# coreperf/rejit

Measured on AMD Instinct MI355X. Metric: GB/s text scanned (regexdna 9 patterns, 50M-line input); matches/s alongside, higher is better.
Workload: dtype u8

## Files before the change

rejit_amd/csrc/kernels.h:

```cpp
#ifndef REJIT_AMD_KERNELS_H_
#define REJIT_AMD_KERNELS_H_

#include <hip/hip_runtime.h>
#include <stdint.h>

#include "dense_streams.h"
#include "device_program.h"
#include "run_scan.h"

namespace rejit_amd {

enum { kCntCands = 0, kCntFinal = 1, kCntOverflow = 2, kCntAdjacent = 3, kCntHits = 4, kCntMaxRegion = 5, kCntOverrun = 6,
  kCntUnordered = 7,
  kCntConflict = 8,
  kCntSharedMax = 9,
  kCntLongWalks = 10,
  kCntSlowStarts = 11,
  kCntSize = 12 };
constexpr uint32_t kOgcMaxBlocks = 256;
constexpr size_t kCounterBlockWords = kCntSize + 2 * kOgcMaxBlocks;
static_assert(kCntLongWalks - kCntOverrun == kLongWalksAfterOverrun, "rj_lane_longest finds the long-walk counter behind the overrun flag");

constexpr uint64_t kNoMatch = ~0ull;

// ... 106 lines not shown
  int n_lists;
  const uint64_t* spans[kMaxFused];
  uint64_t count[kMaxFused];
};
void launch_first_last(const BoundsParams& a, uint64_t* pinned_bounds, hipStream_t st);
void launch_bounds_rows(const BoundsParams& a, int64_t offset, int first_round, int64_t* d_rows, hipStream_t st);
void launch_carry_decide(const int64_t* d_all, int world, int rank, int n_patterns, int64_t* out, hipStream_t st);
void launch_globalize_spans(const uint64_t* local, uint64_t count, int64_t offset, uint64_t* out, hipStream_t st);
void launch_scan_windows_fused(const FusedParams& a, int grid, hipEvent_t t0, hipEvent_t t1, hipStream_t st);

struct PlaneParams {
  const uint8_t* text;
  uint64_t n;
  uint64_t sb, se;
  uint64_t span_pairs;
  uint32_t offset;
  uint32_t code_shift;
  uint32_t n_bases;
  uint32_t lo[2][8], hi[2][8];
  uint64_t* hits;
  uint32_t region_cap;
  uint32_t* hit_counts;
  uint32_t n_zero;
  unsigned long long* zero_counters[kMaxFused];
};
void launch_plane_scan(const PlaneParams& a, int grid, hipEvent_t t0, hipEvent_t t1, hipStream_t st);

enum { kPcConflict = 1,
       kPcVoid = 2 };
constexpr uint32_t kPcBounds = 0;
constexpr uint32_t kPcTotals = kPcBounds + 64;
constexpr uint32_t kPcFinishGroups = 8;
constexpr uint32_t kPcTicket = kPcTotals + 32;
constexpr uint32_t kPcGroupRows = kPcTicket + 16;
constexpr uint32_t kPcAccWords = kPcGroupRows + kPcFinishGroups * 96;
constexpr uint32_t kPcHostCount = 0, kPcHostFlags = 32, kPcHostBounds = 40, kPcHostWords = 40 + 64;
constexpr unsigned long long kPcNone = ~0ull;
constexpr uint32_t kPcLenShift = 56;
struct PlaneCountParams {
  const uint8_t* text;
  uint64_t n;
  uint64_t sb, se;
  uint64_t first_block, end_block;
  uint64_t span_blocks;
  uint32_t span_extra;
  uint32_t code_shift, n_bases, n_patterns;
  uint32_t batch_at;
  uint32_t mask_bits;
  uint32_t base_lo[2], base_hi[2];
  const uint32_t* table;
  uint32_t table_words;
  unsigned long long* acc;
  uint32_t* wg_rows;
  unsigned long long* wg_bounds;
  unsigned long long* host_out;
};
void launch_plane_count(const PlaneCountParams& a, int grid, hipEvent_t t0, hipEvent_t t1, hipStream_t st);
struct PlaneListParams {
  PlaneCountParams c;
  uint64_t* hits;
  uint32_t region_cap;
  uint32_t offset;
  uint32_t* hit_counts;
  uint32_t n_zero;
  unsigned long long* zero_counters[kMaxFused];
};
void launch_plane_list(const PlaneListParams& a, int grid, hipEvent_t t0, hipEvent_t t1, hipStream_t st);
void launch_plane_count_finish(const PlaneCountParams& a, int grid, hipStream_t st);
void launch_bounds_rows_counts(const BoundsParams& a, const unsigned long long* acc, int64_t offset, int first_round, int64_t* d_rows, hipStream_t st);

struct StreamParams {
  const uint8_t* text;
  uint64_t n;
  uint64_t sb, se;
  uint64_t first_tile, n_tiles;
  unsigned long long* granules;
  unsigned long long* ticket;
  uint64_t* out;
  uint64_t out_cap;
  unsigned long long* counters;
  unsigned long long* host_counters;
  uint32_t max_walk;
  StreamPlan plan;
};
uint64_t stream_tiles(uint64_t sb, uint64_t se, uint64_t n, uint64_t* first_tile);
size_t stream_scratch_bytes(uint64_t n_tiles);
void launch_dense_streams(StreamParams a, unsigned long long* scratch, hipEvent_t t0, hipEvent_t t1, hipStream_t st);

constexpr uint64_t kRunTile = 8192;
struct RunSummary {
// ... 209 lines not shown
```

rejit_amd/csrc/multi_pattern.hip:

```cpp

#include <cstring>
#include <dlfcn.h>

#include <hip/hip_runtime.h>

#include <algorithm>
#include <chrono>
#include <cstdio>
#include <cstdlib>
#include <memory>
#include <mutex>
#include <string>
#include <thread>
#include <vector>

#include "engine_internal.h"
#include "exact_count.h"

using namespace rejit_amd;

#define fail ::rejit_amd::rj_fail

namespace {

// ... 250 lines not shown
  bool classify_tables_ready = false;
  DeviceBuffer dummy_counts;
  DeviceBuffer tails;
  MultiTail* host_tails = nullptr;
  uint64_t* host_bounds = nullptr;
  hipStream_t second = nullptr;
  hipEvent_t fork = nullptr, join = nullptr;
  std::vector<MultiTail> uploaded;
  bool fused = false;
  bool batchable = false;
  int mode = 0;
  float scan_ms = 0.f;
  struct Pending {
    bool active = false;
    int kind = 0;
    const uint8_t* text = nullptr;
    uint64_t n = 0, sb = 0, se = 0;
    hipStream_t st = nullptr;
    bool fuse = false;
    std::vector<uint64_t> caps;
    uint32_t shared_cap = 0;
    hipEvent_t done = nullptr;
  } pending;
  rj_multi* scan_after = nullptr;
  hipStream_t tail_stream = nullptr;
  bool tails_own_stream = false;
  DeviceBuffer exchange_rows;
  int64_t* host_decision = nullptr;
  bool counts_only = false;
  ExactCountPlan exact;
  DeviceBuffer exact_table, count_acc, wg_rows, wg_bounds;
  unsigned long long* count_out = nullptr;
  bool counts_ready = false;
  PlanePlan gplane;
  bool general_counts = false;
  DeviceBuffer count_blob;
  uint32_t count_desc_words = 0, count_blob_words = 0, count_lmax = 0, count_max_short = 0;
  int count_max_words = 1;
  bool count_blob_ready = false;
  bool last_counts = false;
  uint32_t counts_fallbacks = 0;

};

namespace {

SharedHits shared_hits_of(rj_multi* m, const uint8_t* d_text, uint64_t n, uint64_t sb, uint64_t se, uint32_t shared_cap, uint32_t n_regions, int P) {
  SharedHits sh{};
  sh.hits = m->shared_hits.as<uint64_t>();
  sh.counts = m->shared_counts.as<uint32_t>();
  sh.cap = shared_cap;
  sh.n_regions = n_regions;
  sh.n_patterns = static_cast<uint32_t>(P);
  sh.win_offset = m->plane.offset;
  sh.text = d_text;
  sh.n = n;
  sh.sb = sb;
  sh.se = se;
  static const bool forward = getenv("RJ_CLASSIFY_FORWARD") != nullptr;
  sh.reverse = forward ? 0u : 1u;
  return sh;
}

int classify_blob(rj_multi* m, hipStream_t st) {
  const int P = static_cast<int>(m->scans.size());
  if (!m->host_desc) RJ_HIP(hipHostMalloc(reinterpret_cast<void**>(&m->host_desc), sizeof(ClassifyDesc) * kMaxFused));
// ... 566 lines not shown
  RJ_HIP(hipStreamSynchronize(st));
  m->count_blob_ready = true;
  return RJ_OK;
}

int run_spans(rj_multi* m, const uint8_t* d_text, uint64_t n, uint64_t sb, uint64_t se, hipStream_t st) {
  if (m->fused && m->mode == 0 && n >= 16) {
    int rc = run_batched(m, d_text, n, sb, se, st, true);
    if (rc != kRegionsFull) return rc != RJ_OK ? rc : 1;
  } else if (m->batchable && n >= 16) {
    int rc = run_batched(m, d_text, n, sb, se, st, false);
    if (rc != kRegionsFull) return rc != RJ_OK ? rc : 2;
  }
  for (rj_scan* s : m->scans) {
    int rc = run_pipeline(s, d_text, n, sb, se, 0, 0, 0, st);
    if (rc != RJ_OK) return rc;
  }
  return 0;
}

int run_counts(rj_multi* m, const uint8_t* d_text, uint64_t n, uint64_t sb, uint64_t se, hipStream_t st, int phase) {
  const int P = static_cast<int>(m->scans.size());
  rj_scan* const s0 = m->scans[0];
  if (phase != 2) {
    const bool general = !(m->exact.ok && m->plane.ok && !m->plane.general && m->plane.offset == 0);
    const PlanePlan& plan = general ? m->gplane : m->plane;
    const uint32_t cmp = general ? plan.n_cmp : 8u;
    const uint64_t last_w = n >= cmp ? n - cmp + 1 : 0;
    const uint64_t wlo = sb + (general ? plan.min_offset : 0u), whi = std::min<uint64_t>(se + (general ? plan.max_offset : 0u), last_w);
    const uint64_t first_block = wlo / 2048;
    const uint64_t end_block = whi > wlo ? (whi + 2047) / 2048 : first_block;
    const uint64_t blocks = end_block - first_block;
    static const int count_chunks = getenv("RJ_COUNT_CHUNKS") ? atoi(getenv("RJ_COUNT_CHUNKS")) : 128;
    const ScanGeometry geo = scan_geometry(std::max<uint64_t>(blocks * 2, 1), static_cast<uint64_t>(count_chunks > 0 ? count_chunks : 128));
    if (!m->counts_ready) {
      if (!m->count_out) RJ_HIP(hipHostMalloc(reinterpret_cast<void**>(&m->count_out), sizeof(unsigned long long) * kPcHostWords));
      if (m->exact.ok) {
        RJ_HIP(m->exact_table.reserve(sizeof(uint32_t) * kExactTabWords));
        RJ_HIP(hipMemcpyAsync(m->exact_table.p, m->exact.table, sizeof(uint32_t) * kExactTabWords, hipMemcpyHostToDevice, st));
      }
      RJ_HIP(m->count_acc.reserve(sizeof(unsigned long long) * kPcAccWords));
      RJ_HIP(hipMemsetAsync(m->count_acc.p, 0, sizeof(unsigned long long) * kPcAccWords, st));
      m->counts_ready = true;
    }
    PlaneCountParams pc{};
    pc.text = d_text;
    pc.n = n;
    pc.sb = sb;
    pc.se = se;
    pc.first_block = first_block;
    pc.end_block = end_block;
    pc.span_blocks = blocks / geo.n_regions;
    pc.span_extra = static_cast<uint32_t>(blocks % geo.n_regions);
    pc.code_shift = plan.code_shift;
    pc.n_bases = plan.n_bases;
    pc.n_patterns = static_cast<uint32_t>(P);
    static const int batch_at = getenv("RJ_COUNT_BATCH") ? atoi(getenv("RJ_COUNT_BATCH")) : 64;
    pc.batch_at = static_cast<uint32_t>(std::min(std::max(batch_at, 1), 64));
    PlaneCountGParams pg{};
    if (general) {
      int rc = count_blob(m, st);
      if (rc != RJ_OK) return rc;
      pc.table = m->count_blob.as<uint32_t>();
      pc.table_words = m->count_blob_words;
      pg.n_cmp = plan.n_cmp;
      pg.tolerance = plan.tolerance;
      pg.lmax = m->count_lmax;
      pg.desc_words = m->count_desc_words;
      for (uint32_t b = 0; b < kPlaneMaxBases; b++)
        for (uint32_t i = 0; i < 8; i++)
          pg.idx[b][i] = i < plan.n_cmp ? (static_cast<uint32_t>(plan.base[b < plan.n_bases ? b : 0][i]) >> plan.code_shift) & 3u : 4u;
    } else {
      for (uint32_t b = 0; b < 2; b++) {
        const uint32_t bb = b < plan.n_bases ? b : 0;
        for (int i = 0; i < 8; i++) {
          const uint32_t code = (static_cast<uint32_t>(plan.base[bb][i]) >> plan.code_shift) & 3u;
          if (!(code & 1u)) pc.mask_bits |= 1u << (16 * b + 2 * i);
          if (!(code & 2u)) pc.mask_bits |= 1u << (16 * b + 2 * i + 1);
        }
        pc.base_lo[b] = m->exact.base_lo[bb];
        pc.base_hi[b] = m->exact.base_hi[bb];
      }
      pc.table = m->exact_table.as<uint32_t>();
    }
    pc.acc = m->count_acc.as<unsigned long long>();
    pc.host_out = m->count_out;
    RJ_HIP(m->wg_rows.reserve(sizeof(uint32_t) * kExactMaxPatterns * static_cast<size_t>(geo.grid)));
    RJ_HIP(m->wg_bounds.reserve(sizeof(unsigned long long) * 2 * kExactMaxPatterns * static_cast<size_t>(geo.grid)));
    pc.wg_rows = m->wg_rows.as<uint32_t>();
    pc.wg_bounds = m->wg_bounds.as<unsigned long long>();
    if (m->scan_after != nullptr && m->scan_after != m && m->scan_after->scans[0]->ev[2] != nullptr)
      RJ_HIP(hipStreamWaitEvent(st, m->scan_after->scans[0]->ev[2], 0));
    if (general) {
      pg.c = pc;
      launch_plane_count_general(pg, m->count_max_words, m->count_max_short, geo.grid, s0->t0(), s0->ev[2], st);
    } else {
      launch_plane_count(pc, geo.grid, s0->t0(), s0->ev[2], st);
    }
    hipStream_t fs = st;
    if (phase == 1) {
      if (!m->tail_stream) RJ_HIP(hipStreamCreateWithFlags(&m->tail_stream, hipStreamNonBlocking));
      fs = m->tail_stream;
      RJ_HIP(hipStreamWaitEvent(fs, s0->ev[2], 0));
    }
    launch_plane_count_finish(pc, geo.grid, fs);
    if (phase == 1) {
      if (!m->pending.done) RJ_HIP(hipEventCreateWithFlags(&m->pending.done, hipEventDisableTiming));
      RJ_HIP(hipEventRecord(m->pending.done, fs));
      return RJ_OK;
    }
  }
  if (phase == 2) RJ_HIP(hipEventSynchronize(m->pending.done));
  else RJ_HIP(hipStreamSynchronize(st));
  RJ_HIP(hipGetLastError());
  if (m->count_out[kPcHostFlags] != 0) {
    m->counts_fallbacks++;
    m->last_counts = false;
    int kind = run_spans(m, d_text, n, sb, se, st);
    return kind < 0 ? kind : RJ_OK;
  }
  m->scan_ms = 0.f;
  if (s0->timing) (void)hipEventElapsedTime(&m->scan_ms, s0->ev[1], s0->ev[2]);
  for (int p = 0; p < P; p++) {
    rj_scan* s = m->scans[static_cast<size_t>(p)];
    s->stats = rj_stats{};
    s->result = nullptr;
    s->result_count = m->count_out[kPcHostCount + p];
    s->stats.n_matches = s->result_count;
    s->stats.scan_ms = m->scan_ms;
    s->stats.count_path = 1;
// ... 452 lines not shown
int64_t rj_scan_gather_spans(rj_scan* s, const void* d_text, uint64_t n, uint64_t own_begin, uint64_t own_end, int64_t offset, void* rccl_comm, int rank,
                             int world, int root, void* hip_stream) {
  if (!rccl_comm) return fail(RJ_BAD_ARGUMENT, "rj_scan_gather_spans: no communicator");
  if (!rccl().all_gather) return fail(RJ_DEVICE_ERROR, "rj_scan_gather_spans: librccl.so not found (set RJ_RCCL_LIBRARY)");
  RcclGatherCtx c{rccl_comm, rank, world};
  return rj_scan_gather_spans_via(s, d_text, n, own_begin, own_end, offset, rccl_allgather_ctx, rccl_gatherv, &c, rank, world, root, hip_stream);
}

const uint64_t* rj_scan_gathered_spans(const rj_scan* s, uint64_t* count) {
  if (count) *count = s ? s->gathered_count : 0;
  return s ? s->gathered : nullptr;
}

int rj_multi_set_tail_stream(rj_multi* m, int on) {
  ErrnoGuard errno_guard;
  if (!m) return fail(RJ_BAD_ARGUMENT, "null argument");
  if (m->pending.active) return fail(RJ_BAD_ARGUMENT, "rj_multi_set_tail_stream: a run is in flight");
  if (on && !m->tail_stream) RJ_HIP(hipStreamCreateWithFlags(&m->tail_stream, hipStreamNonBlocking));
  m->tails_own_stream = on != 0;
  return RJ_OK;
}

int rj_multi_set_timing(rj_multi* m, int on) {
  if (!m) return fail(RJ_BAD_ARGUMENT, "null argument");
  for (rj_scan* s : m->scans) s->timing = on != 0;
  return RJ_OK;
}

int rj_multi_set_counts_only(rj_multi* m, int on) {
  ErrnoGuard errno_guard;
  if (!m) return fail(RJ_BAD_ARGUMENT, "null argument");
  if (m->pending.active) return fail(RJ_BAD_ARGUMENT, "rj_multi_set_counts_only: a run is in flight");
  m->counts_only = on != 0;
  return (m->counts_only && counts_shape(m)) ? 1 : 0;
}

}

int64_t rejit_amd::scan_count(rj_scan* s, const uint8_t* d_text, uint64_t n, hipStream_t st) {
  s->rec_valid = false;
  if (s->counter_state == 0) {
    s->counter_state = -1;
    const rj_program* progs[1] = {s->prog};
    rj_multi* m = nullptr;
    if (n >= 16 && (fusable(s->prog) || plane_general_ok(s->prog)) && rj_multi_create(progs, 1, &m) == RJ_OK) {
      if (rj_multi_set_counts_only(m, 1) == 1) {
        (void)rj_multi_set_timing(m, s->timing ? 1 : 0);
        s->counter = m;
        s->counter_state = 1;
      } else {
        rj_multi_destroy(m);
      }
    } else if (n < 16) {
      s->counter_state = 0;
    }
  }
  if (s->counter_state == 1 && n >= 16 && (reinterpret_cast<uintptr_t>(d_text) & 15u) == 0) {
    uint64_t count = 0;
    int how = rj_multi_run(s->counter, d_text, n, &count, st);
    if (how < 0) return how;
    rj_scan* inner = s->counter->scans[0];
    s->stats = inner->stats;
    s->result_count = inner->result_count;
    s->result = nullptr;
    if (how != 3) s->stats.count_path = 0;
    return static_cast<int64_t>(count);
// ... 25 lines not shown
```

rejit_amd/csrc/plane_count.hip:

```cpp
#include <hip/hip_runtime.h>
#include <hip/hip_ext.h>

#include <cstdlib>

#include "exact_count.h"
#include "kernels.h"
#include "plane_codes.h"
#include "short_walk.h"
#include "stream_load.h"
#include "wave_ops.h"

namespace rejit_amd {

namespace {

constexpr uint64_t kBlock = 2048;
constexpr uint32_t kPieceB = 1024;
constexpr uint32_t kStashWords = (2048 + 16) / 4;
#ifndef RJ_PC_RING
#define RJ_PC_RING 256
#endif
constexpr uint32_t kRing = RJ_PC_RING;

__device__ __forceinline__ uint32_t codes16(const uint4& v, const PlaneCodes& k) {
// ... 119 lines not shown
        const uint32_t e = E[i][b];
        if (i == 0) {
          Z[b] = e;
        } else if (i == 1) {
          O[b] = Z[b] | e;
          Z[b] &= e;
        } else {
          O[b] = Z[b] | (O[b] & e);
          if (i < 7) Z[b] &= e;
        }
      }
  }
  return NB > 1 ? (O[0] | O[NB - 1]) : O[0];
}


struct Lens {
  uint64_t w[2];
};
static_assert(kMaxFused <= 24, "two words of twelve lengths");
__device__ __forceinline__ uint32_t len_of(const Lens& l, uint32_t p) {
  return static_cast<uint32_t>((p < 12 ? l.w[0] >> (5 * p) : l.w[1] >> (5 * (p - 12))) & 31u);
}

}

template <int NB>
struct ExactShape {
  using Args = PlaneCountParams;
  static constexpr uint32_t kFixedLen = 8;
  static constexpr bool kBlobInLds = false;
  static constexpr bool kList = false;
  static constexpr bool kCapture = true;
  __device__ static __forceinline__ const PlaneCountParams& common(const Args& g) { return g; }
  __device__ static __forceinline__ uint32_t lmax(const Args&) { return 8u; }
  __device__ static __forceinline__ uint32_t offset_of(const Args&, const uint32_t*, uint32_t) { return 0u; }
  __device__ static __forceinline__ uint32_t test(uint32_t ta, uint32_t tb, uint32_t ha, uint32_t hb, const Args& g) { return plane_test<NB>(ta, tb, ha, hb, g); }
  __device__ static __forceinline__ void classify(const Args& a, const uint32_t* table, uint64_t pos, bool have, uint32_t& mask, Lens&) {
    const bool ok = have && pos >= a.sb && pos < a.se && pos + 8 <= a.n;
    uint32_t lo = 0, hi = 0;
    if (ok) {
      __builtin_memcpy(&lo, a.text + pos, 4);
      __builtin_memcpy(&hi, a.text + pos + 4, 4);
    }
    mask = exact_classify<NB>(table, a.base_lo, a.base_hi, lo, hi);
    mask = ok ? mask : 0u;
  }
  __device__ static __forceinline__ void classify_bytes(const Args& a, const uint32_t* table, uint64_t pos, bool have, uint32_t lo, uint32_t hi, uint32_t& mask) {
    const bool ok = have && pos >= a.sb && pos < a.se && pos + 8 <= a.n;
    mask = exact_classify<NB>(table, a.base_lo, a.base_hi, lo, hi);
    mask = ok ? mask : 0u;
  }
};

template <int NB>
struct ListShape {
  using Args = PlaneListParams;
  static constexpr uint32_t kFixedLen = 8;
  static constexpr bool kBlobInLds = false;
  static constexpr bool kList = true;
  static constexpr bool kCapture = false;
  __device__ static __forceinline__ void classify_bytes(const Args&, const uint32_t*, uint64_t, bool, uint32_t, uint32_t, uint32_t& mask) { mask = 0; }
  __device__ static __forceinline__ const PlaneCountParams& common(const Args& g) { return g.c; }
  __device__ static __forceinline__ uint32_t lmax(const Args&) { return 8u; }
  __device__ static __forceinline__ uint32_t offset_of(const Args&, const uint32_t*, uint32_t) { return 0u; }
  __device__ static __forceinline__ uint32_t test(uint32_t ta, uint32_t tb, uint32_t ha, uint32_t hb, const Args& g) { return plane_test<NB>(ta, tb, ha, hb, g.c); }
  __device__ static __forceinline__ void classify(const Args&, const uint32_t*, uint64_t, bool, uint32_t& mask, Lens&) { mask = 0; }
};

namespace {

template <bool TOL>
__device__ __forceinline__ uint32_t general_test(uint32_t ta, uint32_t tb, uint32_t ha, uint32_t hb, const PlaneCountGParams& g) {
  constexpr uint32_t kEven = 0x55555555u;
  const uint32_t L = (ta & kEven) | ((tb << 1) & ~kEven);
  const uint32_t H = ((ta >> 1) & kEven) | (tb & ~kEven);
  const uint32_t Ln = (ha & kEven) | ((hb << 1) & ~kEven);
  const uint32_t Hn = ((ha >> 1) & kEven) | (hb & ~kEven);
  register uint32_t q0 asm("v48") = ~(L | H);
  register uint32_t q1 asm("v49") = L & ~H;
  register uint32_t q2 asm("v50") = ~L & H;
  register uint32_t q3 asm("v51") = L & H;
  register uint32_t q4 asm("v52") = ~0u;
  register uint32_t n0 asm("v56") = ~(Ln | Hn);
  register uint32_t n1 asm("v57") = Ln & ~Hn;
  register uint32_t n2 asm("v58") = ~Ln & Hn;
  register uint32_t n3 asm("v59") = Ln & Hn;
  register uint32_t n4 asm("v60") = ~0u;
  uint32_t c = 0;
#pragma clang loop unroll(disable)
  for (uint32_t b = 0; b < g.c.n_bases; b++) {
    const uint32_t* ix = g.idx[b];
    uint32_t e0, e1, e2, e3, e4, e5, e6, e7;
    asm volatile(
// ... 19 lines not shown
          "v"(q3), "v"(q4), "v"(n0), "v"(n1), "v"(n2), "v"(n3), "v"(n4));
    if (TOL) {
      uint32_t Z = e0, O = e0 | e1;
      Z &= e1;
      O = Z | (O & e2);
      Z &= e2;
      O = Z | (O & e3);
      Z &= e3;
      O = Z | (O & e4);
      Z &= e4;
      O = Z | (O & e5);
      Z &= e5;
      O = Z | (O & e6);
      Z &= e6;
      O = Z | (O & e7);
      c |= O;
    } else {
      const uint32_t z0 = e0 & e1 & e2, z1 = e3 & e4 & e5;
      c |= z0 & z1 & e6 & e7;
    }
  }
  return c;
}

}

template <int W, int MAXK, bool TOL>
struct GeneralShape {
  using Args = PlaneCountGParams;
  static constexpr uint32_t kFixedLen = 0;
  static constexpr bool kBlobInLds = true;
  static constexpr bool kList = false;
  static constexpr bool kCapture = false;
  __device__ static __forceinline__ void classify_bytes(const Args&, const uint32_t*, uint64_t, bool, uint32_t, uint32_t, uint32_t& mask) { mask = 0; }
  __device__ static __forceinline__ const PlaneCountParams& common(const Args& g) { return g.c; }
  __device__ static __forceinline__ uint32_t lmax(const Args& g) { return g.lmax; }
  __device__ static __forceinline__ uint32_t offset_of(const Args&, const uint32_t* blob, uint32_t p) {
    return reinterpret_cast<const ClassifyDesc*>(blob)[p].win_offset;
  }
  __device__ static __forceinline__ uint32_t test(uint32_t ta, uint32_t tb, uint32_t ha, uint32_t hb, const Args& g) { return general_test<TOL>(ta, tb, ha, hb, g); }
  __device__ static __forceinline__ void classify(const Args& g, const uint32_t* blob, uint64_t w, bool have, uint32_t& mask, Lens& lens) {
    const PlaneCountParams& a = g.c;
    const ClassifyDesc* desc = reinterpret_cast<const ClassifyDesc*>(blob);
    const uint32_t* tab = blob + g.desc_words;
    uint32_t lo = 0, hi = 0;
    if (have) {
      if (w + 8 <= a.n) {
        __builtin_memcpy(&lo, a.text + w, 4);
        __builtin_memcpy(&hi, a.text + w + 4, 4);
      } else {
        for (uint32_t q = 0; q < 8 && w + q < a.n; q++) {
          const uint32_t c = a.text[w + q];
          if (q < 4) lo |= c << (8 * q);
          else hi |= c << (8 * (q - 4));
        }
      }
    }
    uint32_t todo = 0;
    for (uint32_t p = 0; p < a.n_patterns; p++) {
      const ClassifyDesc& d = desc[p];
      const uint64_t s = w - d.win_offset;
      const bool ok = have && w >= d.win_offset && s >= a.sb && s < a.se && w + d.win_len <= a.n;
      bool win = false;
      for (uint32_t q = 0; q < d.n_windows; q++) win = win || ((((lo ^ d.v0[q]) & d.m0[q]) | ((hi ^ d.v1[q]) & d.m1[q])) == 0);
      todo |= (ok && win) ? 1u << p : 0u;
    }
    mask = 0;
    lens.w[0] = lens.w[1] = 0;
    while (__ballot(todo != 0) != 0) {
      const bool act = todo != 0;
      const uint32_t p = act ? static_cast<uint32_t>(__builtin_ctz(todo)) : 0u;
      todo &= todo - 1;
      const ClassifyDesc& d = desc[p];
      const uint32_t* t0 = tab + d.tab;
      const uint64_t s = w - d.win_offset;
      uint64_t t_lo = 0, t_hi = 0;
      if (act) rj_load16(a.text, a.n, s, &t_lo, &t_hi);
      const uint32_t avail = act ? (a.n - s < 16 ? static_cast<uint32_t>(a.n - s) : 16u) : 0u;
      uint32_t len = 0;
      bool found;
      if (W == 1 || d.n_words <= 1) found = short_longest_lds<1, MAXK>(t0, d, t_lo, t_hi, avail, &len);
      else found = short_longest_lds<W, MAXK>(t0, d, t_lo, t_hi, avail, &len);
      if (found && act && len != 0) {
        mask |= 1u << p;
        if (p < 12) lens.w[0] |= static_cast<uint64_t>(len) << (5 * p);
        else lens.w[1] |= static_cast<uint64_t>(len) << (5 * (p - 12));
      }
    }
  }
};

template <bool TOL>
struct GeneralListShape {
  using Args = PlaneListGParams;
  static constexpr uint32_t kFixedLen = 0;
  static constexpr bool kBlobInLds = false;
  static constexpr bool kList = true;
  static constexpr bool kCapture = false;
  __device__ static __forceinline__ void classify_bytes(const Args&, const uint32_t*, uint64_t, bool, uint32_t, uint32_t, uint32_t& mask) { mask = 0; }
  __device__ static __forceinline__ const PlaneCountParams& common(const Args& g) { return g.g.c; }
  __device__ static __forceinline__ uint32_t lmax(const Args& g) { return g.g.lmax; }
  __device__ static __forceinline__ uint32_t offset_of(const Args&, const uint32_t*, uint32_t) { return 0u; }
  __device__ static __forceinline__ uint32_t test(uint32_t ta, uint32_t tb, uint32_t ha, uint32_t hb, const Args& g) { return general_test<TOL>(ta, tb, ha, hb, g.g); }
  __device__ static __forceinline__ void classify(const Args&, const uint32_t*, uint64_t, bool, uint32_t& mask, Lens&) { mask = 0; }
};

namespace {

struct WaveState {
  uint32_t* ring;
  uint32_t* stash;
  uint32_t head, tail;
  uint32_t acc;
  uint32_t flags;
  uint32_t prev_rel, prev_valid;
  uint32_t* ends;
  uint64_t* list;
  uint32_t list_cap;
  uint64_t list_base;
};
constexpr uint32_t kNoEnd = 0xFFFFFFFFu;

template <bool LIST, bool CAPTURE>
__device__ __forceinline__ void push_block(WaveState& w, uint32_t hm, uint32_t rel_lane, uint32_t block_rel = 0, uint32_t slot = 0) {
  const uint64_t any = __ballot(hm != 0);
  if (any == 0) return;
  auto put = [&](uint32_t idx, uint32_t rel) {
    if (LIST) {
      if (idx < w.list_cap) w.list[idx] = w.list_base + rel;
    } else {
      w.ring[idx & (kRing - 1)] = rel;
// ... 107 lines not shown
  uint32_t any[2] = {0, 0};
#pragma unroll
  for (int round = 0; round < 2; round++) {
    const uint64_t pos = round == 0 ? span_base + static_cast<uint64_t>(lane) - reach : span_base + rel;
    const bool mine = round == 0 ? (static_cast<uint32_t>(lane) < reach && span_base + static_cast<uint64_t>(lane) >= reach) : near;
    uint32_t mask;
    Lens lens;
    S::classify(g, tab, pos, mine, mask, lens);
    for (uint32_t p = 0; p < a.n_patterns; p++)
      if (__ballot(((mask >> p) & 1u) != 0) != 0) any[round] |= 1u << p;
  }
  if ((any[0] & any[1]) != 0) w.flags |= kPcConflict;
}

template <class S>
__device__ __forceinline__ void blocks_done(WaveState& w, const uint32_t* tab, const typename S::Args& g, uint64_t span_base, bool& first_batch) {
  const PlaneCountParams& a = S::common(g);
  if (w.tail - w.head > kRing) {
    w.flags |= kPcVoid;
    w.head = w.tail;
    return;
  }
  while (w.tail - w.head >= a.batch_at) {
    const uint32_t held = w.tail - w.head;
    const uint32_t m = held < 64u ? held : 64u;
    if (first_batch) check_span_start<S>(w, m, tab, g, span_base);
    first_batch = false;
    classify_batch<S>(w, m, tab, g, span_base);
  }
}

}

template <class S>
__global__ __launch_bounds__(256) void plane_count(typename S::Args g) {
  __shared__ __attribute__((aligned(16))) uint32_t table[kExactTabWords];
  extern __shared__ __attribute__((aligned(16))) uint32_t blob[];
  __shared__ uint32_t rings[4][kRing * (S::kCapture ? 3 : 1)];
  __shared__ __attribute__((aligned(16))) uint32_t stashes[4][S::kCapture ? 2 * kStashWords : 4];
  __shared__ uint32_t ends[4][4 * kExactMaxPatterns];
  __shared__ unsigned long long wave_bounds[4][kExactMaxPatterns][2];
  __shared__ uint32_t wave_counts[4][kExactMaxPatterns];
  __shared__ uint32_t wave_flags[4];
  const PlaneCountParams& a = S::common(g);
  const uint32_t* tab = S::kBlobInLds ? blob : table;
  const int lane = lane_id();
  const uint32_t wid = threadIdx.x >> 6;
  const uint32_t wave = __builtin_amdgcn_readfirstlane(static_cast<uint32_t>((static_cast<uint64_t>(blockIdx.x) * blockDim.x + threadIdx.x) >> 6));
  PlaneCodes k;
  k.shift = a.code_shift;
  k.cmask = 0x03030303u << a.code_shift;
  const uint32_t c0 = static_cast<uint32_t>(a.first_block) + wave * static_cast<uint32_t>(a.span_blocks) + (wave < a.span_extra ? wave : a.span_extra);
  const uint32_t c1 = c0 + static_cast<uint32_t>(a.span_blocks) + (wave < a.span_extra ? 1u : 0u);
  const uint32_t full = static_cast<uint32_t>(a.n / kBlock);
  uint32_t fast_end = full >= 1 ? full - 1 : 0;
  if (fast_end > c1) fast_end = c1;
  if (fast_end < c0) fast_end = c0;
  const uint64_t span_base = static_cast<uint64_t>(c0) * kBlock;
  WaveState w;
  w.ring = rings[wid];
  w.stash = stashes[wid];
  w.ends = ends[wid];
  w.head = w.tail = 0;
  w.acc = 0;
  w.flags = 0;
  w.prev_rel = w.prev_valid = 0;
  w.ends[lane] = kNoEnd;
  w.ends[lane + 64] = kNoEnd;
  w.list = nullptr;
  w.list_cap = 0;
  w.list_base = 0;
  if constexpr (S::kList) {
    if (wave == 0 && lane < kCntSize)
      for (uint32_t p = 0; p < g.n_zero; p++) g.zero_counters[p][lane] = 0;
    w.list = g.hits + static_cast<uint64_t>(wave) * g.region_cap;
    w.list_cap = g.region_cap;
    w.list_base = span_base - g.offset;
  }
  bool first_batch = true;

  const uint32_t last_own = fast_end > c0 ? fast_end - 1 : c0;
  auto blk = [&](uint32_t c) { return a.text + static_cast<uint64_t>(c < last_own ? c : last_own) * kBlock; };
  const uint32_t lane_rel = static_cast<uint32_t>(lane) * 16u;
  Raw ra, rb;
  uint2 behind{0, 0};
  uint32_t c = c0;
  auto stash_put = [&](uint32_t ci, const Raw& r) __attribute__((always_inline)) {
    if constexpr (S::kCapture) {
      uint32_t* sl = w.stash + (ci & 1u) * kStashWords;
      *reinterpret_cast<uint4*>(sl + lane * 4) = r.a;
      *reinterpret_cast<uint4*>(sl + kPieceB / 4 + lane * 4) = r.b;
    }
  };
  auto spill_put = [&](uint32_t ci, uint32_t x, uint32_t y) __attribute__((always_inline)) {
    if constexpr (S::kCapture) {
      if (lane == 0) *reinterpret_cast<uint2*>(w.stash + (ci & 1u) * kStashWords + kBlock / 4) = make_uint2(x, y);
    }
  };
  if (c < fast_end) {
    load_block(blk(c), lane_rel, ra);
    load_block(blk(c + 1), lane_rel, rb);
    behind = *reinterpret_cast<const uint2*>(a.text + static_cast<uint64_t>(fast_end) * kBlock);
  }
  if (S::kList) {
  } else if (S::kBlobInLds) {
    const uint4* src = reinterpret_cast<const uint4*>(a.table);
    uint4* dst = reinterpret_cast<uint4*>(blob);
    for (uint32_t i = threadIdx.x; i < a.table_words / 4; i += blockDim.x) dst[i] = src[i];
  } else {
    for (uint32_t i = threadIdx.x; i < kExactTabWords; i += blockDim.x) table[i] = a.table[i];
  }
  __syncthreads();
  if (c < fast_end) {
    uint32_t xa = codes16(ra.a, k), xb = codes16(ra.b, k);
    stash_put(c, ra);
    if (S::kCapture) __builtin_amdgcn_sched_barrier(0);
    load_block(blk(c + 2), lane_rel, ra);
    const uint32_t behind_codes = (codes4(behind.x, k) >> k.shift) | (codes4(behind.y, k) << (8 - k.shift));
    while (c + 1 < fast_end) {
      const uint32_t ya = codes16(rb.a, k), yb = codes16(rb.b, k);
      asm volatile("" ::"v"(ya), "v"(yb));
      stash_put(c + 1, rb);
      spill_put(c, rb.a.x, rb.a.y);
      if (S::kCapture) __builtin_amdgcn_sched_barrier(0);
      if (c + 3 <= last_own) load_block(blk(c + 3), lane_rel, rb);
      {
        const uint32_t ha = wave_from_lane_above(xa, static_cast<uint32_t>(__builtin_amdgcn_readfirstlane(static_cast<int>(xb))));
        const uint32_t hb = wave_from_lane_above(xb, static_cast<uint32_t>(__builtin_amdgcn_readfirstlane(static_cast<int>(ya))));
        const uint32_t hm = S::test(xa, xb, ha, hb, g);
        push_block<S::kList, S::kCapture>(w, hm, (c - c0) * static_cast<uint32_t>(kBlock) + lane_rel, (c - c0) * static_cast<uint32_t>(kBlock), c & 1u);
      }
      __builtin_amdgcn_sched_barrier(0);
      xa = codes16(ra.a, k);
      xb = codes16(ra.b, k);
      asm volatile("" ::"v"(xa), "v"(xb));
      if (c + 2 < fast_end) {
        stash_put(c + 2, ra);
        spill_put(c + 1, ra.a.x, ra.a.y);
      } else {
        spill_put(c + 1, behind.x, behind.y);
      }
      if (S::kCapture) __builtin_amdgcn_sched_barrier(0);
      if (c + 4 <= last_own) load_block(blk(c + 4), lane_rel, ra);
      {
        const uint32_t next0 = c + 2 == fast_end ? behind_codes : static_cast<uint32_t>(__builtin_amdgcn_readfirstlane(static_cast<int>(xa)));
// ... 30 lines not shown
    const uint32_t g0 = guarded_dword(a.text, a.n, at + 16), g1 = guarded_dword(a.text, a.n, at + 20);
    const uint32_t h0 = guarded_dword(a.text, a.n, bt + 16), h1 = guarded_dword(a.text, a.n, bt + 20);
    const uint32_t ha = (codes4(g0, k) >> k.shift) | (codes4(g1, k) << (8 - k.shift));
    const uint32_t hb = (codes4(h0, k) >> k.shift) | (codes4(h1, k) << (8 - k.shift));
    const uint32_t hm = S::test(codes16(va, k), codes16(vb, k), ha, hb, g);
    if (!S::kList && w.tail - w.head > kRing - 64u) blocks_done<S>(w, tab, g, span_base, first_batch);
    if constexpr (S::kCapture) {
      Raw gr;
      gr.a = va;
      gr.b = vb;
      stash_put(c, gr);
      const uint64_t nb = (static_cast<uint64_t>(c) + 1) * kBlock;
      spill_put(c, guarded_dword(a.text, a.n, nb), guarded_dword(a.text, a.n, nb + 4));
    }
    push_block<S::kList, S::kCapture>(w, hm, (c - c0) * static_cast<uint32_t>(kBlock) + lane_rel, (c - c0) * static_cast<uint32_t>(kBlock), c & 1u);
  }
  if constexpr (S::kList) {
    if (lane == 0) g.hit_counts[wave] = w.tail;
    return;
  }
  if (w.tail - w.head > kRing) {
    w.flags |= kPcVoid;
    w.head = w.tail;
  }
  while (w.tail != w.head) {
    const uint32_t held = w.tail - w.head;
    const uint32_t m = held < 64u ? held : 64u;
    if (first_batch) check_span_start<S>(w, m, tab, g, span_base);
    first_batch = false;
    classify_batch<S>(w, m, tab, g, span_base);
  }
  if (lane < kExactMaxPatterns) {
    const bool real = lane < static_cast<int>(a.n_patterns);
    wave_counts[wid][lane] = real ? w.acc : 0u;
    const uint32_t ef = w.ends[4 * lane], efl = w.ends[4 * lane + 1], el = w.ends[4 * lane + 2], ell = w.ends[4 * lane + 3];
    const uint64_t off = real ? S::offset_of(g, tab, static_cast<uint32_t>(lane)) : 0u;
    wave_bounds[wid][lane][0] = ef != kNoEnd ? ((span_base + ef - off) | (static_cast<unsigned long long>(efl) << kPcLenShift)) : kPcNone;
    wave_bounds[wid][lane][1] = ef != kNoEnd ? ((span_base + el - off) | (static_cast<unsigned long long>(ell) << kPcLenShift)) : kPcNone;
  }
  if (lane == 0) wave_flags[wid] = w.flags;
  __syncthreads();
  if (wid != 0 || lane >= kExactMaxPatterns) return;
  uint32_t v = wave_counts[0][lane] + wave_counts[1][lane] + wave_counts[2][lane] + wave_counts[3][lane];
  if (lane == kExactMaxPatterns - 1) v = wave_flags[0] | wave_flags[1] | wave_flags[2] | wave_flags[3];
  a.wg_rows[static_cast<uint64_t>(blockIdx.x) * kExactMaxPatterns + lane] = v;
  if (lane < static_cast<int>(a.n_patterns) && v != 0) {
    unsigned long long first = kPcNone, last = kPcNone;
#pragma unroll
    for (int q = 3; q >= 0; q--)
      if (wave_bounds[q][lane][0] != kPcNone) first = wave_bounds[q][lane][0];
#pragma unroll
    for (int q = 0; q < 4; q++)
      if (wave_bounds[q][lane][1] != kPcNone) last = wave_bounds[q][lane][1];
    *reinterpret_cast<ulonglong2*>(a.wg_bounds + (static_cast<uint64_t>(blockIdx.x) * kExactMaxPatterns + lane) * 2) = ulonglong2{first, last};
  }
}

constexpr uint32_t kFinishBatch = 8;
__global__ __launch_bounds__(256, 8) void plane_count_finish(PlaneCountParams a, uint32_t n_wg) {
  __shared__ unsigned long long part[32][kExactMaxPatterns];
  __shared__ uint32_t part_first[32][kExactMaxPatterns], part_last[32][kExactMaxPatterns];
  __shared__ uint32_t is_last;
  const uint32_t p4 = threadIdx.x & 7u, q = threadIdx.x >> 3;
  const uint32_t per = (n_wg + gridDim.x - 1) / gridDim.x;
  const uint32_t r_lo = blockIdx.x * per, r_hi = r_lo + per < n_wg ? r_lo + per : n_wg;
  uint32_t sum[4] = {0, 0, 0, 0};
  uint32_t first_row[4] = {0, 0, 0, 0}, last_row[4] = {0, 0, 0, 0};
  const uint4* rows = reinterpret_cast<const uint4*>(a.wg_rows);
  for (uint32_t r = r_lo + q; r < r_hi; r += 32 * kFinishBatch) {
    uint4 v[kFinishBatch];
#pragma unroll
    for (uint32_t i = 0; i < kFinishBatch; i++) {
      const uint32_t rr = r + 32 * i;
      v[i] = rows[static_cast<uint64_t>(rr < r_hi ? rr : r) * 8 + p4];
      if (rr >= r_hi) v[i] = uint4{0, 0, 0, 0};
    }
#pragma unroll
    for (uint32_t i = 0; i < kFinishBatch; i++) {
      const uint32_t rr1 = r + 32 * i + 1;
      const uint32_t c[4] = {v[i].x, v[i].y, v[i].z, v[i].w};
      sum[0] += v[i].x;
      sum[1] += v[i].y;
      sum[2] += v[i].z;
      sum[3] = p4 == 7 ? (sum[3] | v[i].w) : (sum[3] + v[i].w);
#pragma unroll
      for (int k = 0; k < 4; k++) {
        first_row[k] = (c[k] != 0 && first_row[k] == 0) ? rr1 : first_row[k];
        last_row[k] = c[k] != 0 ? rr1 : last_row[k];
      }
    }
  }
#pragma unroll
  for (int i = 0; i < 4; i++) {
    part[q][4 * p4 + i] = sum[i];
    part_first[q][4 * p4 + i] = first_row[i];
    part_last[q][4 * p4 + i] = last_row[i];
  }
  __syncthreads();
  const uint32_t lane = threadIdx.x & 63u, wave_id = threadIdx.x >> 6;
  if (wave_id == 0) {
    if (lane < kExactMaxPatterns) {
      unsigned long long t = 0;
      uint32_t f = 0, l = 0;
#pragma unroll 4
      for (uint32_t i = 0; i < 32; i++) {
        t = lane == kExactMaxPatterns - 1 ? (t | part[i][lane]) : (t + part[i][lane]);
        const uint32_t pf = part_first[i][lane], pl = part_last[i][lane];
        f = pf != 0 && (f == 0 || pf < f) ? pf : f;
        l = pl > l ? pl : l;
      }
      unsigned long long* g = a.acc + kPcGroupRows + blockIdx.x * 96;
      __hip_atomic_store(&g[lane], t, __ATOMIC_RELAXED, __HIP_MEMORY_SCOPE_AGENT);
      __hip_atomic_store(&g[32 + lane], static_cast<unsigned long long>(f), __ATOMIC_RELAXED, __HIP_MEMORY_SCOPE_AGENT);
      __hip_atomic_store(&g[64 + lane], static_cast<unsigned long long>(l), __ATOMIC_RELAXED, __HIP_MEMORY_SCOPE_AGENT);
    }
    if (lane == 0) {
      const unsigned long long t = __hip_atomic_fetch_add(&a.acc[kPcTicket], 1ull, __ATOMIC_ACQ_REL, __HIP_MEMORY_SCOPE_AGENT);
      is_last = t + 1 == gridDim.x ? 1u : 0u;
      if (t + 1 == gridDim.x) __hip_atomic_store(&a.acc[kPcTicket], 0ull, __ATOMIC_RELAXED, __HIP_MEMORY_SCOPE_AGENT);
    }
  }
  __syncthreads();
  if (!is_last || threadIdx.x >= kExactMaxPatterns) return;
  const uint32_t p = threadIdx.x;
  unsigned long long total = 0;
  uint32_t f = 0, l = 0;
#pragma unroll 2
  for (uint32_t g = 0; g < gridDim.x; g++) {
    const unsigned long long* row = a.acc + kPcGroupRows + g * 96;
    const unsigned long long v = __hip_atomic_load(&row[p], __ATOMIC_RELAXED, __HIP_MEMORY_SCOPE_AGENT);
    const uint32_t pf = static_cast<uint32_t>(__hip_atomic_load(&row[32 + p], __ATOMIC_RELAXED, __HIP_MEMORY_SCOPE_AGENT));
    const uint32_t pl = static_cast<uint32_t>(__hip_atomic_load(&row[64 + p], __ATOMIC_RELAXED, __HIP_MEMORY_SCOPE_AGENT));
    total = p == kExactMaxPatterns - 1 ? (total | v) : (total + v);
    f = pf != 0 && (f == 0 || pf < f) ? pf : f;
    l = pl > l ? pl : l;
  }
  if (p == kExactMaxPatterns - 1) a.host_out[kPcHostFlags] = total;
  if (p >= a.n_patterns) return;
  unsigned long long first = kPcNone, last = kPcNone;
  if (total != 0 && f != 0) {
    first = a.wg_bounds[(static_cast<uint64_t>(f - 1) * kExactMaxPatterns + p) * 2];
    last = a.wg_bounds[(static_cast<uint64_t>(l - 1) * kExactMaxPatterns + p) * 2 + 1];
  }
  a.host_out[kPcHostCount + p] = total;
  a.host_out[kPcHostBounds + 2 * p] = first;
  a.host_out[kPcHostBounds + 2 * p + 1] = last;
  a.acc[kPcBounds + 2 * p] = first;
  a.acc[kPcBounds + 2 * p + 1] = last;
  a.acc[kPcTotals + p] = total;
}

__global__ void bounds_rows_counts_kernel(BoundsParams a, const unsigned long long* acc, int64_t offset, int first_round, int64_t* rows) {
// ... 4 lines not shown
  if (a.spans[p]) {
    const uint64_t* r = a.spans[p];
    if (n) {
      fb = static_cast<int64_t>(r[0]) + offset;
      fe = static_cast<int64_t>(r[1]) + offset;
      lb = static_cast<int64_t>(r[2 * (n - 1)]) + offset;
      le = static_cast<int64_t>(r[2 * (n - 1) + 1]) + offset;
    }
  } else {
    n = acc[kPcTotals + p];
    if (n) {
      const unsigned long long f = acc[kPcBounds + 2 * p], l = acc[kPcBounds + 2 * p + 1];
      const unsigned long long at = (1ull << kPcLenShift) - 1;
      fb = static_cast<int64_t>(f & at) + offset;
      fe = fb + static_cast<int64_t>(f >> kPcLenShift);
      lb = static_cast<int64_t>(l & at) + offset;
      le = lb + static_cast<int64_t>(l >> kPcLenShift);
    }
  }
  rows[8 * p + 0] = static_cast<int64_t>(n);
  if (first_round) {
    rows[8 * p + 1] = fb;
    rows[8 * p + 2] = fe;
    rows[8 * p + 5] = rows[8 * p + 6] = rows[8 * p + 7] = 0;
  }
  rows[8 * p + 3] = lb;
  rows[8 * p + 4] = le;
}

void launch_bounds_rows_counts(const BoundsParams& a, const unsigned long long* acc, int64_t offset, int first_round, int64_t* d_rows, hipStream_t st) {
  hipLaunchKernelGGL(bounds_rows_counts_kernel, dim3(1), dim3(64), 0, st, a, acc, offset, first_round, d_rows);
}

void launch_plane_count(const PlaneCountParams& a, int grid, hipEvent_t t0, hipEvent_t t1, hipStream_t st) {
  static const size_t pad = getenv("RJ_COUNT_LDS_PAD") ? static_cast<size_t>(atoi(getenv("RJ_COUNT_LDS_PAD"))) : 0;
  if (a.n_bases <= 1) hipExtLaunchKernelGGL((plane_count<ExactShape<1>>), dim3(grid), dim3(256), pad, st, t0, t1, 0, a);
  else hipExtLaunchKernelGGL((plane_count<ExactShape<2>>), dim3(grid), dim3(256), pad, st, t0, t1, 0, a);
}

void launch_plane_list(const PlaneListParams& a, int grid, hipEvent_t t0, hipEvent_t t1, hipStream_t st) {
  if (a.c.n_bases <= 1) hipExtLaunchKernelGGL((plane_count<ListShape<1>>), dim3(grid), dim3(256), 0, st, t0, t1, 0, a);
  else hipExtLaunchKernelGGL((plane_count<ListShape<2>>), dim3(grid), dim3(256), 0, st, t0, t1, 0, a);
}

void launch_plane_list_general(const PlaneListGParams& a, int grid, hipEvent_t t0, hipEvent_t t1, hipStream_t st) {
  if (a.g.tolerance) hipExtLaunchKernelGGL((plane_count<GeneralListShape<true>>), dim3(grid), dim3(256), 0, st, t0, t1, 0, a);
  else hipExtLaunchKernelGGL((plane_count<GeneralListShape<false>>), dim3(grid), dim3(256), 0, st, t0, t1, 0, a);
}

void launch_plane_count_general(const PlaneCountGParams& g, int max_words, uint32_t max_short, int grid, hipEvent_t t0, hipEvent_t t1, hipStream_t st) {
  const size_t lds = static_cast<size_t>(g.c.table_words) * sizeof(uint32_t);
  const dim3 gr(grid), b(256);
  if (g.tolerance) {
    if (max_words <= 1 && max_short <= 8) hipExtLaunchKernelGGL((plane_count<GeneralShape<1, 8, true>>), gr, b, lds, st, t0, t1, 0, g);
    else if (max_words <= 1) hipExtLaunchKernelGGL((plane_count<GeneralShape<1, 16, true>>), gr, b, lds, st, t0, t1, 0, g);
    else hipExtLaunchKernelGGL((plane_count<GeneralShape<2, 16, true>>), gr, b, lds, st, t0, t1, 0, g);
  } else {
    if (max_words <= 1 && max_short <= 8) hipExtLaunchKernelGGL((plane_count<GeneralShape<1, 8, false>>), gr, b, lds, st, t0, t1, 0, g);
    else if (max_words <= 1) hipExtLaunchKernelGGL((plane_count<GeneralShape<1, 16, false>>), gr, b, lds, st, t0, t1, 0, g);
    else hipExtLaunchKernelGGL((plane_count<GeneralShape<2, 16, false>>), gr, b, lds, st, t0, t1, 0, g);
  }
}

void launch_plane_count_finish(const PlaneCountParams& a, int grid, hipStream_t st) {
  hipLaunchKernelGGL(plane_count_finish, dim3(kPcFinishGroups), dim3(256), 0, st, a, static_cast<uint32_t>(grid));
}

}
```

Before: 50230.

## Make exact count kernel persistent with atomic work-unit claiming

The exact plane_count kernel becomes a persistent kernel. Only as many workgroups as fit resident on the device are launched, and each one claims further work units through an atomic counter, double-buffering its per-wave shared reductions across turns. The lookup table is staged into LDS once per workgroup rather than once per unit. The aim is to cut launch and tail cost and to balance load across CUs, at the price of an atomic per unit and a loop with extra state. The claim counter is reset by the finish kernel. Optional env knobs set the unit size, cap the group count, or turn claiming off.

Measured after the change: 41700. -17.0%, worse.

```diff
diff --git a/rejit_amd/csrc/kernels.h b/rejit_amd/csrc/kernels.h
--- a/rejit_amd/csrc/kernels.h
+++ b/rejit_amd/csrc/kernels.h
@@ -162,6 +162,7 @@
 constexpr uint32_t kPcTotals = kPcBounds + 64;
 constexpr uint32_t kPcFinishGroups = 8;
 constexpr uint32_t kPcTicket = kPcTotals + 32;
+constexpr uint32_t kPcClaim = kPcTicket + 8;
 constexpr uint32_t kPcGroupRows = kPcTicket + 16;
 constexpr uint32_t kPcAccWords = kPcGroupRows + kPcFinishGroups * 96;
 constexpr uint32_t kPcHostCount = 0, kPcHostFlags = 32, kPcHostBounds = 40, kPcHostWords = 40 + 64;
@@ -184,8 +185,9 @@
   uint32_t* wg_rows;
   unsigned long long* wg_bounds;
   unsigned long long* host_out;
-};
-void launch_plane_count(const PlaneCountParams& a, int grid, hipEvent_t t0, hipEvent_t t1, hipStream_t st);
+  uint32_t n_units;
+};
+void launch_plane_count(const PlaneCountParams& a, int n_units, int max_groups, hipEvent_t t0, hipEvent_t t1, hipStream_t st);
 struct PlaneListParams {
   PlaneCountParams c;
   uint64_t* hits;
diff --git a/rejit_amd/csrc/multi_pattern.hip b/rejit_amd/csrc/multi_pattern.hip
--- a/rejit_amd/csrc/multi_pattern.hip
+++ b/rejit_amd/csrc/multi_pattern.hip
@@ -306,6 +306,8 @@
   DeviceBuffer exact_table, count_acc, wg_rows, wg_bounds;
   unsigned long long* count_out = nullptr;
   bool counts_ready = false;
+  int count_groups = 0, count_unit_kib = 0;
+  bool count_static = false;
   PlanePlan gplane;
   bool general_counts = false;
   DeviceBuffer count_blob;
@@ -938,7 +940,13 @@
     const uint64_t end_block = whi > wlo ? (whi + 2047) / 2048 : first_block;
     const uint64_t blocks = end_block - first_block;
     static const int count_chunks = getenv("RJ_COUNT_CHUNKS") ? atoi(getenv("RJ_COUNT_CHUNKS")) : 128;
-    const ScanGeometry geo = scan_geometry(std::max<uint64_t>(blocks * 2, 1), static_cast<uint64_t>(count_chunks > 0 ? count_chunks : 128));
+    ScanGeometry geo = scan_geometry(std::max<uint64_t>(blocks * 2, 1), static_cast<uint64_t>(count_chunks > 0 ? count_chunks : 128));
+    const bool claim = !general && !m->count_static;
+    if (!general && m->count_unit_kib > 0) {
+      const uint64_t units = std::min<uint64_t>(std::max<uint64_t>(blocks * 2 / static_cast<uint64_t>(m->count_unit_kib), 1), 16384);
+      geo.grid = static_cast<int>(units);
+      geo.n_regions = static_cast<uint32_t>(units * 4);
+    }
     if (!m->counts_ready) {
       if (!m->count_out) RJ_HIP(hipHostMalloc(reinterpret_cast<void**>(&m->count_out), sizeof(unsigned long long) * kPcHostWords));
       if (m->exact.ok) {
@@ -995,13 +1003,14 @@
     RJ_HIP(m->wg_bounds.reserve(sizeof(unsigned long long) * 2 * kExactMaxPatterns * static_cast<size_t>(geo.grid)));
     pc.wg_rows = m->wg_rows.as<uint32_t>();
     pc.wg_bounds = m->wg_bounds.as<unsigned long long>();
+    pc.n_units = claim ? static_cast<uint32_t>(geo.grid) : 0u;
     if (m->scan_after != nullptr && m->scan_after != m && m->scan_after->scans[0]->ev[2] != nullptr)
       RJ_HIP(hipStreamWaitEvent(st, m->scan_after->scans[0]->ev[2], 0));
     if (general) {
       pg.c = pc;
       launch_plane_count_general(pg, m->count_max_words, m->count_max_short, geo.grid, s0->t0(), s0->ev[2], st);
     } else {
-      launch_plane_count(pc, geo.grid, s0->t0(), s0->ev[2], st);
+      launch_plane_count(pc, geo.grid, m->count_groups, s0->t0(), s0->ev[2], st);
     }
     hipStream_t fs = st;
     if (phase == 1) {
@@ -1520,6 +1529,15 @@
   if (!m) return fail(RJ_BAD_ARGUMENT, "null argument");
   if (m->pending.active) return fail(RJ_BAD_ARGUMENT, "rj_multi_set_counts_only: a run is in flight");
   m->counts_only = on != 0;
+  if (m->counts_only) {
+    auto env_int = [](const char* name) {
+      const char* v = getenv(name);
+      return v ? atoi(v) : 0;
+    };
+    m->count_groups = std::max(env_int("RJ_COUNT_GROUPS"), 0);
+    m->count_unit_kib = std::max(env_int("RJ_COUNT_UNIT_KIB"), 0) & ~1;
+    m->count_static = env_int("RJ_COUNT_STATIC") != 0;
+  }
   return (m->counts_only && counts_shape(m)) ? 1 : 0;
 }
 
diff --git a/rejit_amd/csrc/plane_count.hip b/rejit_amd/csrc/plane_count.hip
--- a/rejit_amd/csrc/plane_count.hip
+++ b/rejit_amd/csrc/plane_count.hip
@@ -175,6 +175,7 @@
   static constexpr bool kBlobInLds = false;
   static constexpr bool kList = false;
   static constexpr bool kCapture = true;
+  static constexpr bool kClaim = true;
   __device__ static __forceinline__ const PlaneCountParams& common(const Args& g) { return g; }
   __device__ static __forceinline__ uint32_t lmax(const Args&) { return 8u; }
   __device__ static __forceinline__ uint32_t offset_of(const Args&, const uint32_t*, uint32_t) { return 0u; }
@@ -203,6 +204,7 @@
   static constexpr bool kBlobInLds = false;
   static constexpr bool kList = true;
   static constexpr bool kCapture = false;
+  static constexpr bool kClaim = false;
   __device__ static __forceinline__ void classify_bytes(const Args&, const uint32_t*, uint64_t, bool, uint32_t, uint32_t, uint32_t& mask) { mask = 0; }
   __device__ static __forceinline__ const PlaneCountParams& common(const Args& g) { return g.c; }
   __device__ static __forceinline__ uint32_t lmax(const Args&) { return 8u; }
@@ -288,6 +290,7 @@
   static constexpr bool kBlobInLds = true;
   static constexpr bool kList = false;
   static constexpr bool kCapture = false;
+  static constexpr bool kClaim = false;
   __device__ static __forceinline__ void classify_bytes(const Args&, const uint32_t*, uint64_t, bool, uint32_t, uint32_t, uint32_t& mask) { mask = 0; }
   __device__ static __forceinline__ const PlaneCountParams& common(const Args& g) { return g.c; }
   __device__ static __forceinline__ uint32_t lmax(const Args& g) { return g.lmax; }
@@ -353,6 +356,7 @@
   static constexpr bool kBlobInLds = false;
   static constexpr bool kList = true;
   static constexpr bool kCapture = false;
+  static constexpr bool kClaim = false;
   __device__ static __forceinline__ void classify_bytes(const Args&, const uint32_t*, uint64_t, bool, uint32_t, uint32_t, uint32_t& mask) { mask = 0; }
   __device__ static __forceinline__ const PlaneCountParams& common(const Args& g) { return g.g.c; }
   __device__ static __forceinline__ uint32_t lmax(const Args& g) { return g.g.lmax; }
@@ -526,6 +530,11 @@
 
 }
 
+#ifdef RJ_PC_TIMELINE
+constexpr uint32_t kTimelineUnits = 1u << 16;
+__device__ unsigned long long rj_pc_timeline[kTimelineUnits][4];
+#endif
+
 template <class S>
 __global__ __launch_bounds__(256) void plane_count(typename S::Args g) {
   __shared__ __attribute__((aligned(16))) uint32_t table[kExactTabWords];
@@ -533,17 +542,27 @@
   __shared__ uint32_t rings[4][kRing * (S::kCapture ? 3 : 1)];
   __shared__ __attribute__((aligned(16))) uint32_t stashes[4][S::kCapture ? 2 * kStashWords : 4];
   __shared__ uint32_t ends[4][4 * kExactMaxPatterns];
-  __shared__ unsigned long long wave_bounds[4][kExactMaxPatterns][2];
-  __shared__ uint32_t wave_counts[4][kExactMaxPatterns];
-  __shared__ uint32_t wave_flags[4];
+  constexpr int kTurns = S::kClaim ? 2 : 1;
+  __shared__ unsigned long long wave_bounds[kTurns][4][kExactMaxPatterns][2];
+  __shared__ uint32_t wave_counts[kTurns][4][kExactMaxPatterns];
+  __shared__ uint32_t wave_flags[kTurns][4];
+  __shared__ uint32_t next_unit[kTurns];
   const PlaneCountParams& a = S::common(g);
   const uint32_t* tab = S::kBlobInLds ? blob : table;
   const int lane = lane_id();
   const uint32_t wid = threadIdx.x >> 6;
-  const uint32_t wave = __builtin_amdgcn_readfirstlane(static_cast<uint32_t>((static_cast<uint64_t>(blockIdx.x) * blockDim.x + threadIdx.x) >> 6));
+  const bool claiming = S::kClaim && a.n_units != 0;
+  uint32_t unit = blockIdx.x, turn = 0;
+  bool staged = false;
   PlaneCodes k;
   k.shift = a.code_shift;
   k.cmask = 0x03030303u << a.code_shift;
+  WaveState w;
+  w.ring = rings[wid];
+  w.stash = stashes[wid];
+  w.ends = ends[wid];
+  for (;;) {
+  const uint32_t wave = static_cast<uint32_t>(__builtin_amdgcn_readfirstlane(static_cast<int>(4u * unit + wid)));
   const uint32_t c0 = static_cast<uint32_t>(a.first_block) + wave * static_cast<uint32_t>(a.span_blocks) + (wave < a.span_extra ? wave : a.span_extra);
   const uint32_t c1 = c0 + static_cast<uint32_t>(a.span_blocks) + (wave < a.span_extra ? 1u : 0u);
   const uint32_t full = static_cast<uint32_t>(a.n / kBlock);
@@ -551,10 +570,6 @@
   if (fast_end > c1) fast_end = c1;
   if (fast_end < c0) fast_end = c0;
   const uint64_t span_base = static_cast<uint64_t>(c0) * kBlock;
-  WaveState w;
-  w.ring = rings[wid];
-  w.stash = stashes[wid];
-  w.ends = ends[wid];
   w.head = w.tail = 0;
   w.acc = 0;
   w.flags = 0;
@@ -596,7 +611,18 @@
     load_block(blk(c + 1), lane_rel, rb);
     behind = *reinterpret_cast<const uint2*>(a.text + static_cast<uint64_t>(fast_end) * kBlock);
   }
-  if (S::kList) {
+  uint32_t drawn = 0;
+  if constexpr (S::kClaim) {
+    if (claiming && threadIdx.x == 0) drawn = __builtin_amdgcn_atomic_inc32(reinterpret_cast<uint32_t*>(&a.acc[kPcClaim]), 0xFFFFFFFFu, __ATOMIC_RELAXED, "agent");
+  }
+#ifdef RJ_PC_TIMELINE
+  if (threadIdx.x == 0 && unit < kTimelineUnits) {
+    rj_pc_timeline[unit][0] = wall_clock64();
+    rj_pc_timeline[unit][2] = blockIdx.x;
+  }
+#endif
+  if (staged) {
+  } else if (S::kList) {
   } else if (S::kBlobInLds) {
     const uint4* src = reinterpret_cast<const uint4*>(a.table);
     uint4* dst = reinterpret_cast<uint4*>(blob);
@@ -604,7 +630,8 @@
   } else {
     for (uint32_t i = threadIdx.x; i < kExactTabWords; i += blockDim.x) table[i] = a.table[i];
   }
-  __syncthreads();
+  if (!staged) __syncthreads();
+  staged = true;
   if (c < fast_end) {
     uint32_t xa = codes16(ra.a, k), xb = codes16(ra.b, k);
     stash_put(c, ra);
@@ -701,29 +728,56 @@
   }
   if (lane < kExactMaxPatterns) {
     const bool real = lane < static_cast<int>(a.n_patterns);
-    wave_counts[wid][lane] = real ? w.acc : 0u;
+    wave_counts[turn][wid][lane] = real ? w.acc : 0u;
     const uint32_t ef = w.ends[4 * lane], efl = w.ends[4 * lane + 1], el = w.ends[4 * lane + 2], ell = w.ends[4 * lane + 3];
     const uint64_t off = real ? S::offset_of(g, tab, static_cast<uint32_t>(lane)) : 0u;
-    wave_bounds[wid][lane][0] = ef != kNoEnd ? ((span_base + ef - off) | (static_cast<unsigned long long>(efl) << kPcLenShift)) : kPcNone;
-    wave_bounds[wid][lane][1] = ef != kNoEnd ? ((span_base + el - off) | (static_cast<unsigned long long>(ell) << kPcLenShift)) : kPcNone;
-  }
-  if (lane == 0) wave_flags[wid] = w.flags;
+    wave_bounds[turn][wid][lane][0] = ef != kNoEnd ? ((span_base + ef - off) | (static_cast<unsigned long long>(efl) << kPcLenShift)) : kPcNone;
+    wave_bounds[turn][wid][lane][1] = ef != kNoEnd ? ((span_base + el - off) | (static_cast<unsigned long long>(ell) << kPcLenShift)) : kPcNone;
+  }
+  if (lane == 0) wave_flags[turn][wid] = w.flags;
+  if constexpr (S::kClaim) {
+    if (threadIdx.x == 0) next_unit[turn] = claiming ? gridDim.x + drawn : ~0u;
+  }
   __syncthreads();
-  if (wid != 0 || lane >= kExactMaxPatterns) return;
-  uint32_t v = wave_counts[0][lane] + wave_counts[1][lane] + wave_counts[2][lane] + wave_counts[3][lane];
-  if (lane == kExactMaxPatterns - 1) v = wave_flags[0] | wave_flags[1] | wave_flags[2] | wave_flags[3];
-  a.wg_rows[static_cast<uint64_t>(blockIdx.x) * kExactMaxPatterns + lane] = v;
-  if (lane < static_cast<int>(a.n_patterns) && v != 0) {
-    unsigned long long first = kPcNone, last = kPcNone;
-#pragma unroll
-    for (int q = 3; q >= 0; q--)
-      if (wave_bounds[q][lane][0] != kPcNone) first = wave_bounds[q][lane][0];
-#pragma unroll
-    for (int q = 0; q < 4; q++)
-      if (wave_bounds[q][lane][1] != kPcNone) last = wave_bounds[q][lane][1];
-    *reinterpret_cast<ulonglong2*>(a.wg_bounds + (static_cast<uint64_t>(blockIdx.x) * kExactMaxPatterns + lane) * 2) = ulonglong2{first, last};
-  }
-}
+  if (wid == 0 && lane < kExactMaxPatterns) {
+    uint32_t v = wave_counts[turn][0][lane] + wave_counts[turn][1][lane] + wave_counts[turn][2][lane] + wave_counts[turn][3][lane];
+    if (lane == kExactMaxPatterns - 1) v = wave_flags[turn][0] | wave_flags[turn][1] | wave_flags[turn][2] | wave_flags[turn][3];
+    a.wg_rows[static_cast<uint64_t>(unit) * kExactMaxPatterns + lane] = v;
+    if (lane < static_cast<int>(a.n_patterns) && v != 0) {
+      unsigned long long first = kPcNone, last = kPcNone;
+#pragma unroll
+      for (int q = 3; q >= 0; q--)
+        if (wave_bounds[turn][q][lane][0] != kPcNone) first = wave_bounds[turn][q][lane][0];
+#pragma unroll
+      for (int q = 0; q < 4; q++)
+        if (wave_bounds[turn][q][lane][1] != kPcNone) last = wave_bounds[turn][q][lane][1];
+      *reinterpret_cast<ulonglong2*>(a.wg_bounds + (static_cast<uint64_t>(unit) * kExactMaxPatterns + lane) * 2) = ulonglong2{first, last};
+    }
+  }
+#ifdef RJ_PC_TIMELINE
+  if (threadIdx.x == 0 && unit < kTimelineUnits) rj_pc_timeline[unit][1] = wall_clock64();
+#endif
+  if constexpr (!S::kClaim) {
+    return;
+  } else {
+    if (!claiming) return;
+    unit = static_cast<uint32_t>(__builtin_amdgcn_readfirstlane(static_cast<int>(next_unit[turn])));
+    if (unit >= a.n_units) return;
+    turn ^= 1u;
+  }
+  }
+}
+
+#ifdef RJ_PC_TIMELINE
+extern "C" int rjb_pc_timeline_read(unsigned long long* out, uint32_t units) {
+  return hipMemcpyFromSymbol(out, HIP_SYMBOL(rj_pc_timeline), sizeof(unsigned long long) * 4 * (units < kTimelineUnits ? units : kTimelineUnits)) == hipSuccess ? 0 : -1;
+}
+extern "C" int rjb_pc_timeline_clear() {
+  void* p = nullptr;
+  if (hipGetSymbolAddress(&p, HIP_SYMBOL(rj_pc_timeline)) != hipSuccess) return -1;
+  return hipMemset(p, 0, sizeof(unsigned long long) * 4 * kTimelineUnits) == hipSuccess ? 0 : -1;
+}
+#endif
 
 constexpr uint32_t kFinishBatch = 8;
 __global__ __launch_bounds__(256, 8) void plane_count_finish(PlaneCountParams a, uint32_t n_wg) {
@@ -786,7 +840,10 @@
     if (lane == 0) {
       const unsigned long long t = __hip_atomic_fetch_add(&a.acc[kPcTicket], 1ull, __ATOMIC_ACQ_REL, __HIP_MEMORY_SCOPE_AGENT);
       is_last = t + 1 == gridDim.x ? 1u : 0u;
-      if (t + 1 == gridDim.x) __hip_atomic_store(&a.acc[kPcTicket], 0ull, __ATOMIC_RELAXED, __HIP_MEMORY_SCOPE_AGENT);
+      if (t + 1 == gridDim.x) {
+        __hip_atomic_store(&a.acc[kPcTicket], 0ull, __ATOMIC_RELAXED, __HIP_MEMORY_SCOPE_AGENT);
+        __hip_atomic_store(&a.acc[kPcClaim], 0ull, __ATOMIC_RELAXED, __HIP_MEMORY_SCOPE_AGENT);
+      }
     }
   }
   __syncthreads();
@@ -857,10 +914,35 @@
   hipLaunchKernelGGL(bounds_rows_counts_kernel, dim3(1), dim3(64), 0, st, a, acc, offset, first_round, d_rows);
 }
 
-void launch_plane_count(const PlaneCountParams& a, int grid, hipEvent_t t0, hipEvent_t t1, hipStream_t st) {
+namespace {
+template <class S>
+int resident_groups(size_t dynamic_lds) {
+  static const int groups = [&] {
+    int dev = 0, cus = 0, per_cu = 0;
+    if (hipGetDevice(&dev) != hipSuccess || hipDeviceGetAttribute(&cus, hipDeviceAttributeMultiprocessorCount, dev) != hipSuccess) return 0;
+    if (hipOccupancyMaxActiveBlocksPerMultiprocessor(&per_cu, plane_count<S>, 256, dynamic_lds) != hipSuccess) return 0;
+    return cus * per_cu;
+  }();
+  return groups;
+}
+
+template <class S>
+void launch_exact(const PlaneCountParams& a, int n_units, int max_groups, size_t pad, hipEvent_t t0, hipEvent_t t1, hipStream_t st) {
+  int grid = n_units;
+  if (a.n_units != 0) {
+    int groups = resident_groups<S>(pad);
+    if (groups <= 0) groups = n_units;
+    if (max_groups > 0 && max_groups < groups) groups = max_groups;
+    if (groups < grid) grid = groups;
+  }
+  hipExtLaunchKernelGGL((plane_count<S>), dim3(grid), dim3(256), pad, st, t0, t1, 0, a);
+}
+}
+
+void launch_plane_count(const PlaneCountParams& a, int n_units, int max_groups, hipEvent_t t0, hipEvent_t t1, hipStream_t st) {
   static const size_t pad = getenv("RJ_COUNT_LDS_PAD") ? static_cast<size_t>(atoi(getenv("RJ_COUNT_LDS_PAD"))) : 0;
-  if (a.n_bases <= 1) hipExtLaunchKernelGGL((plane_count<ExactShape<1>>), dim3(grid), dim3(256), pad, st, t0, t1, 0, a);
-  else hipExtLaunchKernelGGL((plane_count<ExactShape<2>>), dim3(grid), dim3(256), pad, st, t0, t1, 0, a);
+  if (a.n_bases <= 1) launch_exact<ExactShape<1>>(a, n_units, max_groups, pad, t0, t1, st);
+  else launch_exact<ExactShape<2>>(a, n_units, max_groups, pad, t0, t1, st);
 }
 
 void launch_plane_list(const PlaneListParams& a, int grid, hipEvent_t t0, hipEvent_t t1, hipStream_t st) {
```
